# NVIDIA/cuopt

Hardware: AMD Instinct MI355X
Metric: pdlp_iterations_per_sec (higher is better)
Workload: dtype f64; 1 GPU; c3: synthetic random sparse LP S(m=1000000,n=1000000,k=10,seed=2), nnz=10000000, longest row 10, CSR fp64/int32, Stable2 preset, tolerances 0 (fixed iteration budget); rows=1000000, cols=1000000, nnz=10000000, parallelism=single GPU

## Files before the change

### cuopt_amd/csrc/kernels_layout_build.hip

```cpp
#include <hip/hip_runtime.h>

#include "pdlp_setup.hpp"
#include "setup_primitives.hpp"

namespace {

__global__ void __launch_bounds__(kT) k_panel_count(const int32_t* __restrict__ row0, const int32_t* __restrict__ off,
                                                    const int32_t* __restrict__ idx, int S, int32_t slab_w, int64_t own_from,
                                                    int32_t* __restrict__ count )
{
  __shared__ int c[16];
  if (threadIdx.x < 16) c[threadIdx.x] = 0;
  __syncthreads();
  const int w = blockIdx.x;
  const int32_t a = row0[w], b = row0[w + 1];
  for (int32_t i = a + threadIdx.x; i < b; i += kT) {
    const int32_t k0 = off[i], k1 = off[i + 1];
    if ((int64_t)(k1 - k0) > own_from) continue;
    int s_cur = -1, run = 0;
    for (int32_t k = k0; k < k1; ++k) {
      const int s2 = idx[k] / slab_w;
      if (s2 != s_cur) {
        if (run) atomicAdd(&c[s_cur], run);
        s_cur = s2, run = 0;
// ... 95 lines not shown
                        const int32_t* d_off, const int32_t* d_idx, const double* d_val, int64_t slab_bytes, bool force)
{
  PanelHost h;
  std::vector<char> is_own;
  int64_t own_nnz = 0, own_from = 0;
  const bool timing = getenv("CUOPT_AMD_TIMING") != nullptr;
  auto t_last = std::chrono::steady_clock::now();
  auto plap = [&](const char* what) {
    if (!timing) return;
    const auto now = std::chrono::steady_clock::now();
    fprintf(stderr, "[cuopt_amd setup]     panels: %-18s %6.2f ms\n", what, 1e3 * std::chrono::duration<double>(now - t_last).count());
    t_last = now;
  };
  if (!panel_plan(&h, rows, cols, h_off, slab_bytes, force, nullptr, &is_own, &own_nnz, &own_from)) return 0;
  plap("plan");
  const int W = h.W, S = h.S;
  const int64_t nnz = h_off[rows];
  h.nnz = (size_t)(nnz - own_nnz), h.rowptr_size = h.seg ? 0 : (size_t)S * ((size_t)rows + W);
  int32_t *row0 = nullptr, *tile_ptr = nullptr, *col = nullptr, *count = nullptr;
  uint16_t* rowptr = nullptr;
  int64_t* rp_base = nullptr;
  TRY(upload_i32(c, &row0, h.row0.data(), h.row0.size()));
  TRY(dev_alloc(c, &count, (size_t)W * S + 1));
  k_panel_count<<<W, kT, 0, c->stream>>>(row0, d_off, d_idx, S, h.slab_w, own_from, count);
  std::vector<int32_t> hc((size_t)W * S);
  HIP_TRY(hipMemcpyAsync(hc.data(), count, hc.size() * sizeof(int32_t), hipMemcpyDeviceToHost, c->stream));
  HIP_TRY(hipStreamSynchronize(c->stream));
  plap("count");
  h.tile_ptr.resize((size_t)W * S + 1);
  int64_t pos = 0;
  for (size_t i = 0; i < (size_t)W * S; ++i) {
    if (!h.seg && hc[i] >= 65536) return 0;
    if (hc[i] >= 65536) return 1;
    h.tile_ptr[i] = (int32_t)pos;
    pos += hc[i];
  }
  h.tile_ptr[(size_t)W * S] = (int32_t)pos;
  h.rp_base.assign((size_t)W * S, 0);
  if (!h.seg)
    for (int w = 0; w < W; ++w) {
      const int64_t a = h.row0[w], nr = h.row0[w + 1] - a, rp = (int64_t)S * (a + w);
      for (int s2 = 0; s2 < S; ++s2) h.rp_base[(size_t)w * S + s2] = rp + (int64_t)s2 * (nr + 1);
    }
  TRY(upload_i32(c, &tile_ptr, h.tile_ptr.data(), h.tile_ptr.size()));
  {
    auto pad = [](size_t b) { return (b + 255) & ~(size_t)255; };
    const size_t b_col = pad((h.nnz + 8) * sizeof(int32_t)), b_rp = pad((h.rowptr_size + 8) * sizeof(uint16_t)), b_val = pad((h.nnz + 8) * sizeof(double));
    char* block = nullptr;
    HIP_TRY(hipMalloc((void**)&block, 2 * b_col + b_rp + b_val));
    c->allocs.push_back(block);
    c->bytes += (int64_t)(2 * b_col + b_rp + b_val);
    dst->val  = (double*)block;
    col       = (int32_t*)(block + b_val);
    dst->perm = (int32_t*)(block + b_val + b_col);
    rowptr    = (uint16_t*)(block + b_val + 2 * b_col);
  }
  TRY(dev_alloc(c, &rp_base, h.rp_base.size()));
  HIP_TRY(hipMemcpyAsync(rp_base, h.rp_base.data(), h.rp_base.size() * sizeof(int64_t), hipMemcpyHostToDevice, c->stream));
  plap("alloc");
  {
    const size_t lds = (size_t)S * (kPanelMaxRows + 1) * sizeof(unsigned short);
    static std::mutex mu;
    static std::vector<int> done;
    {
      std::lock_guard<std::mutex> lock(mu);
      if (std::find(done.begin(), done.end(), c->device) == done.end()) {
        HIP_TRY(hipFuncSetAttribute((const void*)k_panel_place<false>, hipFuncAttributeMaxDynamicSharedMemorySize, 16 * (kPanelMaxRows + 1) * 2));
        HIP_TRY(hipFuncSetAttribute((const void*)k_panel_place<true>, hipFuncAttributeMaxDynamicSharedMemorySize, 16 * (kPanelMaxRows + 1) * 2));
        done.push_back(c->device);
      }
    }
    if (h.seg) k_panel_place<true><<<W, 512, lds, c->stream>>>(row0, d_off, d_idx, S, h.slab_w, own_from, tile_ptr, rp_base, rowptr, dst->perm, col);
    else k_panel_place<false><<<W, 512, lds, c->stream>>>(row0, d_off, d_idx, S, h.slab_w, own_from, tile_ptr, rp_base, rowptr, dst->perm, col);
    HIP_TRY(hipGetLastError());
    if (h.sorted) {
      k_panel_sort<<<W * S, 512, 0, c->stream>>>(S, h.slab_w, tile_ptr, dst->perm, col);
      HIP_TRY(hipGetLastError());
    }
  }
  HIP_TRY(hipStreamSynchronize(c->stream));
  plap("place");
  dst->v = PanelView{h.W, h.S, h.any_long ? 1 : 0, row0, tile_ptr, rowptr, rp_base, col, dst->val};
  dst->v.seg = h.seg ? 1 : 0, dst->v.slab_w = h.slab_w, dst->v.sorted = h.sorted ? 1 : 0;
  dst->nent  = (int64_t)h.nnz;
  if (!h.own_row.empty()) {
    int32_t *own_row = nullptr, *own_ptr = nullptr;
    TRY(upload_i32(c, &own_row, h.own_row.data(), h.own_row.size()));
    TRY(upload_i32(c, &own_ptr, h.own_ptr.data(), h.own_ptr.size()));
    HIP_TRY(hipStreamSynchronize(c->stream));
    dst->v.NP = h.W, dst->v.W = h.W + (int)h.own_row.size();
    dst->v.own_row = own_row, dst->v.own_ptr = own_ptr;
    dst->v.csr_off = d_off, dst->v.csr_idx = d_idx, dst->v.csr_val = d_val;
  }
  dst->on = true;
  return 0;
}

namespace {
constexpr int kPbBinT  = 1024;
constexpr int kPbSortN = 16384;
static_assert(kPbCap <= kPbSortN && kPbMaxRows <= 1024, "a bin's entries / rows fit the LDS sorts");

__global__ void __launch_bounds__(kT) k_max_row_len(int32_t rows, const int32_t* __restrict__ off, int* __restrict__ out)
{
  int best = 0;
  for (int64_t r = (int64_t)blockIdx.x * kT + threadIdx.x; r < rows; r += (int64_t)gridDim.x * kT) best = max(best, off[r + 1] - off[r]);
  for (int d = 1; d < 64; d <<= 1) best = max(best, __shfl_xor(best, d, 64));
  if ((threadIdx.x & 63) == 0 && best > 0) atomicMax(out, best);
}

constexpr int kPbItems = (kPbCap + kPbBinT - 1) / kPbBinT;
template <int MODE>
__global__ void __launch_bounds__(kPbBinT)
k_pb_bin(const int32_t* __restrict__ row0, const int32_t* __restrict__ off, const int32_t* __restrict__ idx, int panel_shift, int gshift, int S, int B,
         int32_t* __restrict__ bin_size, int* __restrict__ maxpad, uint16_t* __restrict__ cnt, const int32_t* __restrict__ pstart,
         const int32_t* __restrict__ bin_e0, int32_t* __restrict__ perm, uint16_t* __restrict__ lidx, int32_t* __restrict__ piece_dst,
         uint16_t* __restrict__ epos)
{
  __shared__ uint32_t w[kPbSortN];
  __shared__ int scratch[kPbBinT / 64 + 1];
  const int b = blockIdx.x, tid = threadIdx.x;
  const int r0 = row0[b], r1 = row0[b + 1];
  const int k0 = off[r0], n = off[r1] - k0;
  int n2 = 1;
  while (n2 < n) n2 <<= 1;
  for (int i = tid; i < n2; i += kPbBinT) w[i] = i < n ? ((uint32_t)(idx[k0 + i] >> panel_shift) << 14 | (uint32_t)i) : 0xFFFFFFFFu;
  __syncthreads();
  lds_bitonic_sort<kPbBinT>(w, n2);
  const int G = 1 << gshift;
  const int p0 = tid * kPbItems;
  int rs[kPbItems];
  int last = 0;
#pragma unroll
  for (int q = 0; q < kPbItems; ++q) {
    const int i = p0 + q;
    const bool start = i < n && (i == 0 || (w[i] >> 14) != (w[i - 1] >> 14));
    last  = start ? i : last;
    rs[q] = last;
  }
  const int before = block_exclusive_max<kPbBinT>(last, scratch);
#pragma unroll
  for (int q = 0; q < kPbItems; ++q) rs[q] = rs[q] > before ? rs[q] : before;
  int padv[kPbItems], sum = 0;
#pragma unroll
  for (int q = 0; q < kPbItems; ++q) {
    const int i = p0 + q;
    const bool end = i < n && (i == n - 1 || (w[i] >> 14) != (w[i + 1] >> 14));
    padv[q] = end ? (G - ((i - rs[q] + 1) & (G - 1))) & (G - 1) : 0;
    sum += padv[q];
  }
  int total = 0;
  int P = block_exclusive_scan<kPbBinT>(sum, scratch, &total);
  if (MODE <= 1) {
    if (tid == 0) {
      bin_size[b] = n + total;
      atomicMax(maxpad, n + total);
    }
    if (MODE == 0) return;
  }
#pragma unroll
  for (int q = 0; q < kPbItems; ++q) {
    const int i = p0 + q;
    if (i < n) {
      const int s_ = (int)(w[i] >> 14), e = (int)(w[i] & 0x3FFF), k = k0 + e;
      const bool end = i == n - 1 || (w[i] >> 14) != (w[i + 1] >> 14);
      if (MODE == 1) {
// ... 1049 lines not shown
```

### cuopt_amd/csrc/kernels_panel.hip

```cpp
#include <hip/hip_runtime.h>

#include "pdlp_kernel_decls.hpp"
#include "pdlp_layouts.hpp"
#include "pdlp_setup.hpp"
#include "spmv_panel.hpp"

template <bool SEG>
__global__ void __launch_bounds__(kPanelThreads)
k_panel_a_dual(PanelView P, const pdlpdev_ctl* __restrict__ ctl, const double* __restrict__ xbar,
               double* __restrict__ y0, double* __restrict__ y1, const double* __restrict__ lo,
               const double* __restrict__ hi, double* __restrict__ sumy, double* __restrict__ part, double* __restrict__ ycopy,
               const p2pdev::Push* __restrict__ push)
{
  if (!loop_active(ctl)) return;
  DualEpilogue e = DualEpilogue::make(ctl, y0, y1, lo, hi, sumy, ycopy, push);
  const bool masked = !SEG && P.zmask != nullptr && (P.zforce != 0 || ctl->zskip != 0);
  if (masked && blockIdx.x == 0 && threadIdx.x == 0)
    __hip_atomic_fetch_add(const_cast<unsigned long long*>(P.zmask) + 2 * ((size_t)(P.zcols + 127) / 128), 1ull, __ATOMIC_RELAXED, __HIP_MEMORY_SCOPE_AGENT);
  panel_block_zs<SEG>(P, xbar, e, part, masked);
  if (push) p2pdev::count_exchange(push);
}

template <bool SEG>
__global__ void __launch_bounds__(kPanelThreads)
// ... 293 lines not shown
    P.tile_ptr[i] = (int32_t)pos;
    pos += count[i];
  }
  P.tile_ptr[(size_t)W * S] = (int32_t)pos;
  P.nnz = (size_t)(nnz - own_nnz), P.rowptr_size = P.seg ? 0 : (size_t)S * ((size_t)rows + W);
  P.perm.reset(P.nnz), P.col.reset(P.nnz);
  if (P.seg) {
    cuopt_amd::parallel_tasks(W, [&](int w) {
      const int32_t a = P.row0[w], b = P.row0[w + 1];
      std::vector<int32_t> cursor(S);
      for (int s2 = 0; s2 < S; ++s2) cursor[s2] = P.tile_ptr[(size_t)w * S + s2];
      for (int32_t i = a; i < b; ++i) {
        if (is_own[i]) continue;
        for (int32_t t = off[i]; t < off[i + 1]; ++t) {
          const int s2    = idx[t] / slab_w;
          const int32_t q = cursor[s2]++;
          P.perm[q] = t, P.col[q] = (int32_t)(((uint32_t)(i - a) << kSegColBits) | (uint32_t)(idx[t] - s2 * slab_w));
        }
      }
    }, nnz);
    P.ok = true;
    return P;
  }
  P.rowptr.reset(P.rowptr_size);
  P.rp_base.resize((size_t)W * S);
  cuopt_amd::parallel_tasks(W, [&](int w) {
    const int32_t a = P.row0[w], b = P.row0[w + 1], nr = b - a;
    const int64_t rp = (int64_t)S * ((int64_t)a + w);
    std::vector<int32_t> cursor(S);
    for (int s2 = 0; s2 < S; ++s2) {
      cursor[s2]                    = P.tile_ptr[(size_t)w * S + s2];
      P.rp_base[(size_t)w * S + s2] = rp + (int64_t)s2 * (nr + 1);
    }
    for (int32_t i = a; i < b; ++i) {
      for (int s2 = 0; s2 < S; ++s2)
        P.rowptr[(size_t)(P.rp_base[(size_t)w * S + s2] + (i - a))] = (uint16_t)(cursor[s2] - P.tile_ptr[(size_t)w * S + s2]);
      if (is_own[i]) continue;
      for (int32_t t = off[i]; t < off[i + 1]; ++t) {
        const int s2 = idx[t] / slab_w;
        const int32_t q = cursor[s2]++;
        P.perm[q] = t, P.col[q] = idx[t];
      }
    }
    for (int s2 = 0; s2 < S; ++s2)
      P.rowptr[(size_t)(P.rp_base[(size_t)w * S + s2] + nr)] = (uint16_t)(cursor[s2] - P.tile_ptr[(size_t)w * S + s2]);
    if (!P.sorted) return;
    std::vector<uint32_t> key;
    std::vector<int32_t> pm;
    for (int s2 = 0; s2 < S; ++s2)
      for (int32_t c0 = P.tile_ptr[(size_t)w * S + s2], t1 = P.tile_ptr[(size_t)w * S + s2 + 1]; c0 < t1; c0 += kPanelChunk) {
        const int32_t len = std::min<int32_t>(kPanelChunk, t1 - c0);
        key.resize((size_t)len), pm.assign(&P.perm[c0], &P.perm[c0] + len);
        for (int32_t i = 0; i < len; ++i) key[i] = ((uint32_t)(P.col[c0 + i] - s2 * slab_w) << 12) | (uint32_t)i;
        std::sort(key.begin(), key.end());
        for (int32_t i = 0; i < len; ++i) {
          const uint32_t slot = key[i] & 0xFFFu;
          P.col[c0 + i] = (int32_t)((slot << kSegColBits) | (key[i] >> 12)), P.perm[c0 + i] = pm[slot];
        }
      }
  }, nnz);
  P.ok = true;
  return P;
}

int upload_panels(pdlpdev_ctx* c, pdlpdev_ctx::Panels* dst, const PanelHost& h, const int32_t* d_off, const int32_t* d_idx,
                         const double* d_val)
{
  if (!h.ok) return 0;
  int32_t *row0 = nullptr, *tile_ptr = nullptr, *col = nullptr;
  uint16_t* rowptr = nullptr;
  int64_t* rp_base = nullptr;
  TRY(upload_i32(c, &row0, h.row0.data(), h.row0.size()));
  TRY(upload_i32(c, &tile_ptr, h.tile_ptr.data(), h.tile_ptr.size()));
  TRY(upload_i32(c, &col, h.col.get(), h.nnz));
  TRY(upload_i32(c, &dst->perm, h.perm.get(), h.nnz));
  TRY(dev_alloc(c, &rowptr, h.rowptr_size));
  HIP_TRY(hipMemcpyAsync(rowptr, h.rowptr.get(), h.rowptr_size * sizeof(uint16_t), hipMemcpyHostToDevice, c->stream));
  TRY(dev_alloc(c, &rp_base, h.rp_base.size()));
  HIP_TRY(hipMemcpyAsync(rp_base, h.rp_base.data(), h.rp_base.size() * sizeof(int64_t), hipMemcpyHostToDevice, c->stream));
  TRY(dev_alloc(c, &dst->val, h.nnz));
  HIP_TRY(hipStreamSynchronize(c->stream));
  dst->v  = PanelView{h.W, h.S, h.any_long ? 1 : 0, row0, tile_ptr, rowptr, rp_base, col, dst->val};
  dst->v.seg = h.seg ? 1 : 0, dst->v.slab_w = h.slab_w, dst->v.sorted = h.sorted ? 1 : 0;
  dst->nent = (int64_t)h.nnz;
  if (!h.own_row.empty()) {
    int32_t *own_row = nullptr, *own_ptr = nullptr;
    TRY(upload_i32(c, &own_row, h.own_row.data(), h.own_row.size()));
    TRY(upload_i32(c, &own_ptr, h.own_ptr.data(), h.own_ptr.size()));
    HIP_TRY(hipStreamSynchronize(c->stream));
    dst->v.NP = h.W, dst->v.W = h.W + (int)h.own_row.size();
    dst->v.own_row = own_row, dst->v.own_ptr = own_ptr;
    dst->v.csr_off = d_off, dst->v.csr_idx = d_idx, dst->v.csr_val = d_val;
  }
  dst->on = true;
  return 0;
}

int pick_layout(pdlpdev_ctx* c, pdlpdev_ctx::MatrixSide* side, const double* vec, double* out)
{
  pdlpdev_ctx::Panels* pn = &side->pan;
  if (!pn->on) return 0;
  hipEvent_t e0, e1;
  HIP_TRY(hipEventCreate(&e0));
  HIP_TRY(hipEventCreate(&e1));
  float ms_stream = 1e30f, ms_panel = 1e30f;
  for (int round = 0; round < 2; ++round)
    for (int which = 0; which < 2; ++which) {
      for (int rep = 0; rep < 4; ++rep) {
        if (rep == 1) HIP_TRY(hipEventRecord(e0, c->stream));
        if (which == 0)
          k_spmv_plain<<<stream_grid(side->nb), kBlock, 0, c->stream>>>(side->nb, side->rb, side->hot.off, side->hot.idx, side->hot.val, vec, out, (const double*)nullptr);
        else
          (pn->v.seg ? k_panel_plain<true> : k_panel_plain<false>)<<<pn->v.W, kPanelThreads, 0, c->stream>>>(pn->v, vec, out);
      }
      HIP_TRY(hipEventRecord(e1, c->stream));
      HIP_TRY(hipEventSynchronize(e1));
      float ms = 0.f;
      HIP_TRY(hipEventElapsedTime(&ms, e0, e1));
      if (which == 0)
        ms_stream = std::min(ms_stream, ms);
      else
        ms_panel = std::min(ms_panel, ms);
    }
  (void)hipEventDestroy(e0), (void)hipEventDestroy(e1);
  if (getenv("CUOPT_AMD_TIMING"))
    fprintf(stderr, "[cuopt_amd setup]   layout %-3s: stream %.1f us, panels %.1f us -> %s\n", side->name, ms_stream * 1e3 / 3,
            ms_panel * 1e3 / 3, ms_stream <= ms_panel ? "stream" : "panels");
  if (ms_stream <= ms_panel) pn->on = false;
  return 0;
}
```

### cuopt_amd/csrc/pdlp_kernels.hpp

```cpp
#pragma once
#include <hip/hip_runtime.h>
#include <stdint.h>


#include "cuopt_amd/pdlp_device.h"

namespace pdlp {

typedef double vec4d __attribute__((ext_vector_type(4)));
typedef int vec4i __attribute__((ext_vector_type(4)));

constexpr int kBlock    = 256;
constexpr int kNnzTile  = 2048;
constexpr int kNnzBlock = kNnzTile - 4;
constexpr int kLongRow  = 128;
constexpr int kMaxRowsPerBlock = 1024;

template <int XOR_MASK>
__device__ __forceinline__ double swizzle_xor(double v)
{
  static_assert(XOR_MASK >= 1 && XOR_MASK <= 16, "ds_swizzle works inside 32 lanes");
  constexpr int pattern = (XOR_MASK << 10) | 0x1F;
  int lo = __double2loint(v), hi = __double2hiint(v);
  lo = __builtin_amdgcn_ds_swizzle(lo, pattern);
// ... 48 lines not shown
  int lo = __double2loint(v), hi = __double2hiint(v);
  lo = __builtin_amdgcn_update_dpp(0, lo, CTRL, 0xf, 0xf, false);
  hi = __builtin_amdgcn_update_dpp(0, hi, CTRL, 0xf, 0xf, false);
  return __hiloint2double(hi, lo);
}
__device__ __forceinline__ double row16_sum(double v)
{
  v = v + dpp_move<0xB1>(v);
  v = v + dpp_move<0x4E>(v);
  v = v + dpp_move<0x141>(v);
  v = v + dpp_move<0x140>(v);
  return v;
}
__device__ __forceinline__ double read_lane(double v, int lane)
{
  const int lo = __builtin_amdgcn_readlane(__double2loint(v), lane);
  const int hi = __builtin_amdgcn_readlane(__double2hiint(v), lane);
  return __hiloint2double(hi, lo);
}
__device__ __forceinline__ double wave_sum_dpp(double v)
{
  v = row16_sum(v);
  return ((read_lane(v, 0) + read_lane(v, 16)) + read_lane(v, 32)) + read_lane(v, 48);
}
template <int NQ, int WAVES>
__device__ __forceinline__ void block_sum_fast(double (&v)[NQ], double* scratch )
{
  static_assert(NQ <= 4 && WAVES <= 16, "one DPP row per quantity");
  const int lane = threadIdx.x & 63, wave = threadIdx.x >> 6;
#pragma unroll
  for (int q = 0; q < NQ; ++q) {
    const double w = wave_sum_dpp(v[q]);
    if (lane == 0) scratch[q * 16 + wave] = w;
  }
  __syncthreads();
  const int q = lane >> 4, i = lane & 15;
  double part = (q < NQ && i < WAVES) ? scratch[q * 16 + i] : 0.0;
  part        = row16_sum(part);
#pragma unroll
  for (int k = 0; k < NQ; ++k) v[k] = read_lane(part, 16 * k);
}

__device__ __forceinline__ double dense_plus(const double* __restrict__ add, int r, double v) { return add ? v + add[r] : v; }

__device__ __forceinline__ bool loop_active(const pdlpdev_ctl* ctl)
{
  return ctl->error == 0 && ctl->steps_taken < ctl->target_steps;
}
__device__ __forceinline__ bool period_reached(const pdlpdev_ctl* ctl) { return ctl->steps_taken >= ctl->target_steps; }
constexpr int kPeriodGuard = 0x100;
__device__ __forceinline__ bool period_guard_skips(const pdlpdev_ctl* ctl, int& arg)
{
  const bool guarded = (arg & kPeriodGuard) != 0;
  arg &= ~kPeriodGuard;
  return guarded && !period_reached(ctl);
}

__device__ __forceinline__ int xcd_remap(int b, int nb)
{
  const int per = (nb + 7) >> 3;
  const int v   = (b & 7) * per + (b >> 3);
  return v;
}



constexpr int kPanelThreads = 512;
constexpr int kPanelChunk   = 4096;
constexpr int kPanelMaxRows = 3584;
constexpr int kPanelWaves   = kPanelThreads / 64;

struct PanelView {
  int W, S;
  int any_long;
  const int32_t* __restrict__ row0;
  const int32_t* __restrict__ tile_ptr;
  const uint16_t* __restrict__ rowptr;
  const int64_t* __restrict__ rp_base;
  const int32_t* __restrict__ col;
  const double* __restrict__ val;
  const double* __restrict__ dense_add = nullptr;
  int seg = 0, slab_w = 0;
  int sorted = 0;
  int NP = 0;
  const int32_t* __restrict__ own_row = nullptr;
  const int32_t* __restrict__ own_ptr = nullptr;
  const int32_t* __restrict__ csr_off = nullptr;
  const int32_t* __restrict__ csr_idx = nullptr;
  const double* __restrict__ csr_val  = nullptr;
  const int32_t* __restrict__ dn_own_seg   = nullptr;
  const int32_t* __restrict__ dn_pan_ptr   = nullptr;
  const int32_t* __restrict__ dn_pan_seg   = nullptr;
  const int32_t* __restrict__ dn_seg_row   = nullptr;
  const int32_t* __restrict__ dn_seg_c0    = nullptr;
  const int32_t* __restrict__ dn_seg_len   = nullptr;
  const int32_t* __restrict__ dn_seg_ptr   = nullptr;
  const double* __restrict__ dn_val        = nullptr;
  const unsigned long long* __restrict__ zmask = nullptr;
  int zcols = 0, zforce = 0;
};
constexpr int kZsQuads        = 1152;
constexpr int kPanelOwnRow = 4096;
constexpr int kPanelDenseSegs = 32;
constexpr long long kPanelNotMine = 0x7FF8C0DEC0DEC0DELL;

constexpr int kPanelPer     = kPanelChunk / kPanelThreads;
constexpr int kPanelRowsPer = (kPanelMaxRows + kPanelThreads - 1) / kPanelThreads;
constexpr int kSegColBits = 20;
constexpr unsigned kSegColMask = (1u << kSegColBits) - 1u;
static_assert(kPanelChunk <= 1 << 12, "a sorted chunk's slot takes the 12 bits beside the column");

constexpr int kJagMaxGroup = 256;
constexpr int kJagBatchRows = 16384;
#ifndef CUOPT_AMD_JAG_U
#define CUOPT_AMD_JAG_U 8
#endif
constexpr int kJagU        = CUOPT_AMD_JAG_U;
constexpr int jag_window(int waves) { return waves == 16 ? 16384 : 8192; }
constexpr size_t jag_lds_bytes(int waves) { return sizeof(double) * (size_t)(jag_window(waves) + waves * kJagMaxGroup); }
constexpr long long kJagNotMine = 0x7FF8C0DEC0DEC0DELL;

struct JagView {
  int rows, waves, ngroups, nblk, nlong;
  const int32_t* __restrict__ row0;
  const int32_t* __restrict__ tile_e;
  const int32_t* __restrict__ tile_sr;
  const uint32_t* __restrict__ sr;
  const uint16_t* __restrict__ slot;
  const double* __restrict__ val;
  const int32_t* __restrict__ win;
  const int32_t* __restrict__ set_ptr;
  const int32_t* __restrict__ set_col;
  const int32_t* __restrict__ lr_ptr;
  const int32_t* __restrict__ lr_row;
  const int32_t* __restrict__ off;
  const int32_t* __restrict__ idx;
  const double* __restrict__ csr_val;
  const double* __restrict__ dense_add = nullptr;
};


constexpr int kPbThreads = 512;
constexpr int kPbCap     = 9088;
constexpr int kPbMaxRows = 1024;
constexpr int kPbKU      = 16;
constexpr size_t kPbLdsBytes = sizeof(double) * (size_t)(kPbCap + kPbMaxRows + 128);
typedef double pb_vec2d __attribute__((ext_vector_type(2)));
constexpr int kPbwRows     = 8192;
constexpr int kPbwStep     = 1024;
constexpr int kPbwThreads  = 1024;
constexpr int kPbwMaxLevel = 6;
constexpr int kPbwAhead    = 4;
constexpr int kPbwMaxSteps = 4096;
constexpr size_t kPbwLdsBytes = sizeof(double) * (size_t)(kPbwRows + 256) + kPbwMaxSteps;

struct PbView {
  int rows, cols, S, B, gshift, panel_shift, nwg;
  const double* __restrict__ val;
  const uint16_t* __restrict__ lidx;
  const int32_t* __restrict__ piece_dst;
  const int32_t* __restrict__ wg_e0;
  const int32_t* __restrict__ wg_panel;
  const int32_t* __restrict__ bin_row0;
  const int32_t* __restrict__ bin_e0;
  const uint32_t* __restrict__ sr;
  const int32_t* __restrict__ bin_grp;
// ... 143 lines not shown
```

### cuopt_amd/csrc/spmv_panel.hpp

```cpp
#pragma once
#include <type_traits>

#include "pdlp_kernels.hpp"

namespace pdlp {

struct PanelChunk {
  int s, c0, c1, t0;
  bool valid;
};
template <int R>
__device__ __forceinline__ void panel_load(const PanelView& P, double (&va)[kPanelPer], int (&ja)[kPanelPer], int c0, int c1)
{
#pragma unroll
  for (int u = 0; u < R; ++u) {
    int k = c0 + threadIdx.x + u * kPanelThreads;
    if (u == R - 1) k = k < c1 ? k : c1 - 1;
    va[u] = __builtin_nontemporal_load(P.val + k);
    ja[u] = __builtin_nontemporal_load(P.col + k);
  }
}
__device__ __forceinline__ void panel_decode(int word, int i, bool sorted, int slab_base, int& col, int& slot)
{
  col  = sorted ? slab_base + (int)((unsigned)word & kSegColMask) : word;
  slot = sorted ? (int)((unsigned)word >> kSegColBits) : i;
}
template <int R>
__device__ __forceinline__ void panel_products(const double* __restrict__ vec, double* prod, const double (&va)[kPanelPer],
                                               const int (&ja)[kPanelPer], int len, bool sorted, int slab_base)
{
  double x[R];
  int slot[R];
#pragma unroll
  for (int u = 0; u < R; ++u) {
    int c;
    panel_decode(ja[u], threadIdx.x + u * kPanelThreads, sorted, slab_base, c, slot[u]);
    x[u] = vec[c];
  }
#pragma unroll
  for (int u = 0; u < R; ++u) {
    const int i = threadIdx.x + u * kPanelThreads;
    if (u < R - 1 || i < len) prod[slot[u]] = va[u] * x[u];
  }
}
template <int R>
__device__ __forceinline__ void panel_products_zs(const double* __restrict__ vec, double* prod, const double (&va)[kPanelPer],
                                                  const int (&ja)[kPanelPer], int len, const unsigned* zbits, int zbase, bool sorted,
                                                  int slab_base)
{
  unsigned w[R];
  int c[R], slot[R];
#pragma unroll
  for (int u = 0; u < R; ++u) {
    panel_decode(ja[u], threadIdx.x + u * kPanelThreads, sorted, slab_base, c[u], slot[u]);
    const int wi = (c[u] >> 5) - zbase;
    w[u]         = wi < kZsQuads * 4 ? zbits[wi] : ~0u;
  }
  double x[R];
#pragma unroll
  for (int u = 0; u < R; ++u) {
    x[u] = 0.0;
    if ((w[u] >> (c[u] & 31)) & 1u) x[u] = vec[c[u]];
  }
#pragma unroll
  for (int u = 0; u < R; ++u) {
    const int i = threadIdx.x + u * kPanelThreads;
    if (u < R - 1 || i < len) prod[slot[u]] = va[u] * x[u];
  }
}
constexpr int kZsPer = (kZsQuads + kPanelThreads - 1) / kPanelThreads;
__device__ __forceinline__ int panel_zs_first_quad(const PanelView& P, int s) { return (int)(((long long)s * P.slab_w) >> 7); }
__device__ __forceinline__ void panel_zs_load(const PanelView& P, int s, uint4 (&st)[kZsPer])
{
  const long long c1 = (long long)(s + 1) * P.slab_w;
  const int last     = (int)(c1 < P.zcols ? c1 : P.zcols) - 1;
  const int q0       = panel_zs_first_quad(P, s);
  int nq             = (last >> 7) - q0 + 1;
  nq                 = nq < kZsQuads ? nq : kZsQuads;
  const uint4* __restrict__ src = reinterpret_cast<const uint4*>(P.zmask) + q0;
#pragma unroll
  for (int k = 0; k < kZsPer; ++k) {
    const int q = threadIdx.x + k * kPanelThreads;
    st[k]       = uint4{0u, 0u, 0u, 0u};
    if (q < nq) st[k] = src[q];
  }
}
__device__ __forceinline__ void panel_zs_store(uint4* zq, const uint4 (&st)[kZsPer])
{
#pragma unroll
  for (int k = 0; k < kZsPer; ++k) {
    const int q = threadIdx.x + k * kPanelThreads;
    if (q < kZsQuads) zq[q] = st[k];
  }
}
#define PANEL_DISPATCH(rounds, CALL) \
  switch (rounds) {                   \
    case 1: CALL(1); break;           \
    case 2: CALL(2); break;           \
    case 3: CALL(3); break;           \
    case 4: CALL(4); break;           \
    case 5: CALL(5); break;           \
    case 6: CALL(6); break;           \
    case 7: CALL(7); break;           \
// ... 80 lines not shown
    const int k = j - D->c0[q];
    if (k >= 0 && k < D->len[q]) add += __builtin_nontemporal_load(P.dn_val + D->ptr[q] + k) * D->y[q];
  }
  return add;
}
template <class Epi>
__device__ __forceinline__ void panel_epilogue_rows(const PanelView& P, Epi& epi, double (&acc)[Epi::NQ > 0 ? Epi::NQ : 1], const double* psum,
                                                    int first, int r0, int nr, const PanelDenseSegs* D, const double* psum2)
{
  for (int r = first; r < nr; r += kPanelThreads)
    if (__double_as_longlong(psum[r]) != kPanelNotMine) {
      double v = psum2 ? psum[r] + psum2[r] : psum[r];
      if (P.dn_pan_ptr) v = v + panel_dense_col(P, D, r0 + r);
      epi.row(r0 + r, dense_plus(P.dense_add, r0 + r, v), acc);
    }
}
template <class Epi>
__device__ __forceinline__ void panel_epilogue_partials(const PanelView& P, double* __restrict__ partials, double (&acc)[Epi::NQ > 0 ? Epi::NQ : 1],
                                                        double* red, int w)
{
  if constexpr (Epi::NQ > 0) {
    block_reduce<typename Epi::Op, Epi::NQ, kPanelWaves>(acc, red);
    if (threadIdx.x == 0) {
#pragma unroll
      for (int q = 0; q < Epi::NQ; ++q) partials[(size_t)q * P.W + w] = acc[q];
    }
  }
}
template <class Epi>
__device__ __forceinline__ void panel_epilogue(const PanelView& P, Epi& epi, double* __restrict__ partials, const double* psum, double* red,
                                               int w, int r0, int nr, const PanelDenseSegs* D,
                                               const double* psum2 = nullptr )
{
  double acc[Epi::NQ > 0 ? Epi::NQ : 1];
#pragma unroll
  for (int q = 0; q < (Epi::NQ > 0 ? Epi::NQ : 1); ++q) acc[q] = Epi::Op::identity();
  panel_epilogue_rows(P, epi, acc, psum, threadIdx.x, r0, nr, D, psum2);
  panel_epilogue_partials<Epi>(P, partials, acc, red, w);
}

constexpr int kPanelEpiDepth = 4;
template <class Epi, class = void>
struct PanelEarlyOps {
  static constexpr bool on = false;
  struct type {};
};
template <class Epi>
struct PanelEarlyOps<Epi, std::void_t<typename Epi::Ops>> {
  static constexpr bool on = true;
  using type = typename Epi::Ops;
};
template <class Epi>
__device__ __forceinline__ void panel_epilogue_request(const Epi& epi, typename Epi::Ops (&pre)[kPanelEpiDepth], int r0, int nr)
{
#pragma unroll
  for (int q = 0; q < kPanelEpiDepth; ++q) {
    int r  = threadIdx.x + q * kPanelThreads;
    r      = r < nr ? r : 0;
    pre[q] = epi.load(r0 + r);
  }
}
template <class Epi>
__device__ __forceinline__ void panel_epilogue_early(const PanelView& P, Epi& epi, double* __restrict__ partials, const double* psum, double* red,
                                                     int w, int r0, int nr, const PanelDenseSegs* D,
                                                     const typename Epi::Ops (&pre)[kPanelEpiDepth], const double* psum2 = nullptr)
{
  double acc[Epi::NQ > 0 ? Epi::NQ : 1];
#pragma unroll
  for (int q = 0; q < (Epi::NQ > 0 ? Epi::NQ : 1); ++q) acc[q] = Epi::Op::identity();
  __builtin_amdgcn_s_waitcnt(0x0F70);
#pragma unroll
  for (int q = 0; q < kPanelEpiDepth; ++q) {
    const int r = threadIdx.x + q * kPanelThreads;
    if (r < nr && __double_as_longlong(psum[r]) != kPanelNotMine) {
      double v = psum2 ? psum[r] + psum2[r] : psum[r];
      if (P.dn_pan_ptr) v = v + panel_dense_col(P, D, r0 + r);
      epi.apply(r0 + r, dense_plus(P.dense_add, r0 + r, v), pre[q], acc);
    }
  }
  panel_epilogue_rows(P, epi, acc, psum, threadIdx.x + kPanelEpiDepth * kPanelThreads, r0, nr, D, psum2);
  panel_epilogue_partials<Epi>(P, partials, acc, red, w);
}

__device__ __forceinline__ void panel_row_sums(const PanelView& P, const unsigned (&ext)[kPanelRowsPer], const double* prod, double* psum,
                                               int nr, int lo, int hi)
{
  if (!P.any_long) {
#pragma unroll
    for (int q = 0; q < kPanelRowsPer; ++q) {
      const int r = threadIdx.x + q * kPanelThreads;
      if (r < nr) {
        int a = (int)(ext[q] & 0xFFFFu), b = (int)(ext[q] >> 16);
        a = a > lo ? a : lo;
        b = b < hi ? b : hi;
        if (a < b) {
          double sum = psum[r];
          for (int k = a; k < b; ++k) sum = sum + prod[k - lo];
          psum[r] = sum;
        }
      }
    }
    return;
  }
  bool any_long = false;
#pragma unroll
  for (int q = 0; q < kPanelRowsPer; ++q) {
    const int r = threadIdx.x + q * kPanelThreads;
    if (r < nr) {
      int a = (int)(ext[q] & 0xFFFFu), b = (int)(ext[q] >> 16);
      a = a > lo ? a : lo;
      b = b < hi ? b : hi;
      if (b - a > kLongRow) {
        any_long = true;
      } else if (a < b) {
        double sum = psum[r];
        for (int k = a; k < b; ++k) sum = sum + prod[k - lo];
        psum[r] = sum;
      }
    }
  }
  if (__ballot(any_long)) {
#pragma unroll
    for (int q = 0; q < kPanelRowsPer; ++q) {
      const int r = threadIdx.x + q * kPanelThreads;
      int a = 0, b = 0;
      if (r < nr) {
        a = (int)(ext[q] & 0xFFFFu), b = (int)(ext[q] >> 16);
        a = a > lo ? a : lo;
        b = b < hi ? b : hi;
      }
      unsigned long long todo = __ballot(b - a > kLongRow);
      while (todo) {
        const int l  = __builtin_ctzll(todo);
        todo &= todo - 1;
        const int la = __builtin_amdgcn_readlane(a, l), lb = __builtin_amdgcn_readlane(b, l);
        double part  = 0.0;
        for (int k = la + (int)(threadIdx.x & 63); k < lb; k += 64) part = part + prod[k - lo];
        part = wave_reduce<SumOp>(part);
        if ((int)(threadIdx.x & 63) == l) psum[r] = psum[r] + part;
      }
    }
  }
}

template <class Epi, bool ZS = false>
__device__ __forceinline__ void panel_spmv_block(const PanelView& P, const double* __restrict__ vec,
                                                 Epi& epi, double* __restrict__ partials, const unsigned long long* zmask = nullptr)
{
  static_assert(kPanelPer == 8, "PANEL_DISPATCH enumerates 1..8 rounds");
  [[maybe_unused]] uint4* zq = nullptr;
  if constexpr (ZS) {
    __shared__ uint4 zq_s[kZsQuads];
    zq = zq_s;
  }
  const bool zon = ZS && zmask != nullptr;
  __shared__ double prod[kPanelChunk];
  __shared__ double psum[kPanelMaxRows];
  __shared__ double red[kPanelWaves * (Epi::NQ > 0 ? Epi::NQ : 1)];
  __shared__ int tile_s[17];
  __shared__ long long base_s[16];
  const int w  = blockIdx.x;
  const int NP = P.NP ? P.NP : P.W;
  if (w >= NP) {
    panel_own_row(P, vec, epi, partials, w, NP, prod);
    return;
  }
  __shared__ PanelDenseSegs dseg;
  const int r0 = P.row0[w], nr = P.row0[w + 1] - r0;
  panel_dense_prepare(P, w, vec, &dseg);
  if (threadIdx.x <= P.S) tile_s[threadIdx.x] = P.tile_ptr[w * P.S + threadIdx.x];
  if (threadIdx.x < P.S) base_s[threadIdx.x] = P.rp_base[w * P.S + threadIdx.x];
  for (int r = threadIdx.x; r < nr; r += kPanelThreads) psum[r] = 0.0;
  __syncthreads();
  if (P.own_ptr)
    for (int q = P.own_ptr[w] + (int)threadIdx.x; q < P.own_ptr[w + 1]; q += kPanelThreads) psum[P.own_row[q] - r0] = __longlong_as_double(kPanelNotMine);
  auto advance = [&](PanelChunk c) -> PanelChunk {
    if (c.valid && c.c1 < tile_s[c.s + 1]) {
      c.c0 = c.c1;
      c.c1 = c.c0 + kPanelChunk < tile_s[c.s + 1] ? c.c0 + kPanelChunk : tile_s[c.s + 1];
      return c;
    }
    int s = c.s + 1;
    while (s < P.S && tile_s[s + 1] == tile_s[s]) ++s;
    c.valid = s < P.S;
    c.s     = s;
    if (c.valid) {
      c.t0 = c.c0 = tile_s[s];
      c.c1 = c.c0 + kPanelChunk < tile_s[s + 1] ? c.c0 + kPanelChunk : tile_s[s + 1];
    }
    return c;
  };
  double va[kPanelPer];
  int ja[kPanelPer];
  unsigned ext_next[kPanelRowsPer], ext[kPanelRowsPer];
#define PANEL_ROUNDS(c) (((c).c1 - (c).c0 + kPanelThreads - 1) / kPanelThreads)
#define PANEL_CALL_LOAD(R) panel_load<R>(P, va, ja, nxt.c0, nxt.c1)
#define PANEL_CALL_PRODUCTS(R) panel_products<R>(vec, prod, va, ja, cur.c1 - cur.c0, P.sorted != 0, cur.s * P.slab_w)
#define PANEL_CALL_PRODUCTS_ZS(R) panel_products_zs<R>(vec, prod, va, ja, cur.c1 - cur.c0, reinterpret_cast<const unsigned*>(zq), panel_zs_first_quad(P, cur.s) << 2, P.sorted != 0, cur.s * P.slab_w)
#define PANEL_REQUEST(c)                                                         \
  if ((c).valid) {                                                               \
    PANEL_DISPATCH(PANEL_ROUNDS(c), PANEL_CALL_LOAD)                             \
    const uint16_t* __restrict__ rp_ = P.rowptr + base_s[(c).s];                 \
    _Pragma("unroll") for (int q = 0; q < kPanelRowsPer; ++q) {                  \
      int r_      = threadIdx.x + q * kPanelThreads;                             \
      r_          = r_ < nr ? r_ : 0;                                            \
      ext_next[q] = (unsigned)rp_[r_] | ((unsigned)rp_[r_ + 1] << 16);           \
    }                                                                            \
  }
  PanelChunk none{-1, 0, 0, 0, false};
  PanelChunk nxt = advance(none);
  PANEL_REQUEST(nxt)
  PanelChunk cur = nxt;
  if (zon && cur.valid) {
    uint4 st[kZsPer];
    panel_zs_load(P, cur.s, st);
    panel_zs_store(zq, st);
  }
  constexpr bool kEarly = PanelEarlyOps<Epi>::on;
  [[maybe_unused]] typename PanelEarlyOps<Epi>::type pre[kPanelEpiDepth];
  [[maybe_unused]] int lo_last = 0, hi_last = 0;
  while (cur.valid) {
    __syncthreads();
    if (zon) { PANEL_DISPATCH(PANEL_ROUNDS(cur), PANEL_CALL_PRODUCTS_ZS) }
    else { PANEL_DISPATCH(PANEL_ROUNDS(cur), PANEL_CALL_PRODUCTS) }
#pragma unroll
    for (int q = 0; q < kPanelRowsPer; ++q) ext[q] = ext_next[q];
    const int lo = cur.c0 - cur.t0, hi = cur.c1 - cur.t0;
    nxt = advance(cur);
    if constexpr (kEarly)
      if (!nxt.valid) {
        lo_last = lo, hi_last = hi;
        break;
      }
    PANEL_REQUEST(nxt)
    __syncthreads();
    if (zon && nxt.valid && nxt.s != cur.s) {
      uint4 st[kZsPer];
      panel_zs_load(P, nxt.s, st);
      panel_row_sums(P, ext, prod, psum, nr, lo, hi);
      panel_zs_store(zq, st);
    } else {
      panel_row_sums(P, ext, prod, psum, nr, lo, hi);
    }
    cur = nxt;
  }
#undef PANEL_REQUEST
#undef PANEL_CALL_PRODUCTS_ZS
#undef PANEL_CALL_PRODUCTS
#undef PANEL_CALL_LOAD
#undef PANEL_ROUNDS
  if constexpr (kEarly) {
    panel_epilogue_request(epi, pre, r0, nr);
    if (cur.valid) {
      __syncthreads();
      panel_row_sums(P, ext, prod, psum, nr, lo_last, hi_last);
    }
    __syncthreads();
    panel_epilogue_early(P, epi, partials, psum, red, w, r0, nr, &dseg, pre);
  } else {
    __syncthreads();
    panel_epilogue(P, epi, partials, psum, red, w, r0, nr, &dseg);
  }
}
template <int CTRL, int ROW_MASK>
__device__ __forceinline__ double seg_dpp(double v)
{
  int lo = __double2loint(v), hi = __double2hiint(v);
  lo = __builtin_amdgcn_update_dpp(0, lo, CTRL, ROW_MASK, 0xf, false);
  hi = __builtin_amdgcn_update_dpp(0, hi, CTRL, ROW_MASK, 0xf, false);
  return __hiloint2double(hi, lo);
}
__device__ __forceinline__ double seg_scan(double S, int lane, int seg0)
{
  double u;
  u = seg_dpp<0x111, 0xf>(S); if ((lane & 15) >= 1 && lane - 1 >= seg0) S = S + u;
  u = seg_dpp<0x112, 0xf>(S); if ((lane & 15) >= 2 && lane - 2 >= seg0) S = S + u;
  u = seg_dpp<0x114, 0xf>(S); if ((lane & 15) >= 4 && lane - 4 >= seg0) S = S + u;
  u = seg_dpp<0x118, 0xf>(S); if ((lane & 15) >= 8 && lane - 8 >= seg0) S = S + u;
  u = seg_dpp<0x142, 0xa>(S); if ((lane & 16) && (lane | 15) - 16 >= seg0) S = S + u;
  u = seg_dpp<0x143, 0xc>(S); if (lane >= 32 && 31 >= seg0) S = S + u;
  return S;
}
__device__ __forceinline__ void seg_emit(double* strip, int row, double v)
{
  __hip_atomic_fetch_add(strip + row, v, __ATOMIC_RELAXED, __HIP_MEMORY_SCOPE_WORKGROUP);
}
struct SegRecord {
  double lsum, rsum;
  int lkey, rkey;
};
template <int R>
__device__ __forceinline__ void seg_load(const PanelView& P, double (&va)[kPanelPer], int (&pk)[kPanelPer], int c0, int c1)
{
#pragma unroll
  for (int u = 0; u < R; ++u) {
    int k = c0 + threadIdx.x + u * kPanelThreads;
    if (u == R - 1) k = k < c1 ? k : c1 - 1;
    va[u] = __builtin_nontemporal_load(P.val + k);
    pk[u] = __builtin_nontemporal_load(P.col + k);
  }
}
template <int R>
__device__ __forceinline__ void seg_rounds(const double* __restrict__ vec, int slab_base, const double (&va)[kPanelPer], const int (&pk)[kPanelPer], int len,
                                           double* psum, SegRecord* rec , int lane)
{
  double x[R];
#pragma unroll
  for (int u = 0; u < R; ++u) x[u] = vec[slab_base + (int)((unsigned)pk[u] & kSegColMask)];
#pragma unroll
  for (int u = 0; u < R; ++u) {
    const int i   = threadIdx.x + u * kPanelThreads;
    const int key = (int)((unsigned)pk[u] >> kSegColBits);
    const double v = (u < R - 1 || i < len) ? va[u] * x[u] : 0.0;
    const int prev = __builtin_amdgcn_update_dpp(-1, key, 0x138, 0xf, 0xf, false);
    const unsigned long long starts = __ballot(key != prev);
    const unsigned long long below  = starts & ((2ull << lane) - 1ull);
    const int seg0                  = 63 - __builtin_clzll(below);
    const double S                  = seg_scan(v, lane, seg0);
    const bool ends                 = lane == 63 || ((starts >> (lane + 1)) & 1ull);
    if (ends) {
      if (seg0 == 0) {
        rec[u].lsum = S, rec[u].lkey = key;
        if (lane == 63) rec[u].rkey = -1;
      } else if (lane == 63) {
        rec[u].rsum = S, rec[u].rkey = key;
      } else {
        seg_emit(psum, key, S);
      }
    }
  }
}
__device__ __forceinline__ void panel_seg_join(const SegRecord* rec , double* psum2, int R, int lane)
{
  const int u = lane >> 3, q = lane & 7;
  const bool on = u < R;
  SegRecord g{0.0, 0.0, 0, -1};
  if (on) g = rec[q * kPanelPer + u];
  const bool single = g.rkey < 0;
// ... 128 lines not shown
```

Before: 6774 iterations/s.

## Issue panel row-extent loads before entry loads and skip unused row slots

Adds a req_order mode, on by default for non-segmented panels, that fetches row-pointer extents before the value and column loads of the next chunk. The entry loads now use clamped byte offsets and load only the rounds each chunk needs. Row-sum and extent work skips the upper row slots when the panel has few rows, and tile-pointer reads are made wave-uniform with readfirstlane. The aim is to cut load-issue latency and wasted work in the SpMV panel loop. The cost is a second instantiation of the loop body, which adds code size and register pressure.

After: 6880 iterations/s (median of 6 runs). +1.6%, better.

```diff
diff --git a/cuopt_amd/csrc/kernels_layout_build.hip b/cuopt_amd/csrc/kernels_layout_build.hip
--- a/cuopt_amd/csrc/kernels_layout_build.hip
+++ b/cuopt_amd/csrc/kernels_layout_build.hip
@@ -201,6 +201,7 @@
   plap("place");
   dst->v = PanelView{h.W, h.S, h.any_long ? 1 : 0, row0, tile_ptr, rowptr, rp_base, col, dst->val};
   dst->v.seg = h.seg ? 1 : 0, dst->v.slab_w = h.slab_w, dst->v.sorted = h.sorted ? 1 : 0;
+  dst->v.req_order = !h.seg && cuopt_amd::tune_int("panel_req_order", 1) != 0 ? 1 : 0;
   dst->nent  = (int64_t)h.nnz;
   if (!h.own_row.empty()) {
     int32_t *own_row = nullptr, *own_ptr = nullptr;
diff --git a/cuopt_amd/csrc/kernels_panel.hip b/cuopt_amd/csrc/kernels_panel.hip
--- a/cuopt_amd/csrc/kernels_panel.hip
+++ b/cuopt_amd/csrc/kernels_panel.hip
@@ -399,6 +399,7 @@
   HIP_TRY(hipStreamSynchronize(c->stream));
   dst->v  = PanelView{h.W, h.S, h.any_long ? 1 : 0, row0, tile_ptr, rowptr, rp_base, col, dst->val};
   dst->v.seg = h.seg ? 1 : 0, dst->v.slab_w = h.slab_w, dst->v.sorted = h.sorted ? 1 : 0;
+  dst->v.req_order = !h.seg && cuopt_amd::tune_int("panel_req_order", 1) != 0 ? 1 : 0;
   dst->nent = (int64_t)h.nnz;
   if (!h.own_row.empty()) {
     int32_t *own_row = nullptr, *own_ptr = nullptr;
diff --git a/cuopt_amd/csrc/pdlp_kernels.hpp b/cuopt_amd/csrc/pdlp_kernels.hpp
--- a/cuopt_amd/csrc/pdlp_kernels.hpp
+++ b/cuopt_amd/csrc/pdlp_kernels.hpp
@@ -154,6 +154,7 @@
   const double* __restrict__ dense_add = nullptr;
   int seg = 0, slab_w = 0;
   int sorted = 0;
+  int req_order = 0;
   int NP = 0;
   const int32_t* __restrict__ own_row = nullptr;
   const int32_t* __restrict__ own_ptr = nullptr;
diff --git a/cuopt_amd/csrc/spmv_panel.hpp b/cuopt_amd/csrc/spmv_panel.hpp
--- a/cuopt_amd/csrc/spmv_panel.hpp
+++ b/cuopt_amd/csrc/spmv_panel.hpp
@@ -19,6 +19,28 @@
     va[u] = __builtin_nontemporal_load(P.val + k);
     ja[u] = __builtin_nontemporal_load(P.col + k);
   }
+}
+__device__ __forceinline__ void panel_load_rounds(const PanelView& P, double (&va)[kPanelPer], int (&ja)[kPanelPer], int c0, int c1, int rounds)
+{
+  unsigned ov[kPanelPer], oc[kPanelPer];
+  const int last = c1 - c0 - 1;
+#pragma unroll
+  for (int u = 0; u < kPanelPer; ++u) {
+    int i = (int)threadIdx.x + u * kPanelThreads;
+    i     = i < last ? i : last;
+    ov[u] = (unsigned)i * 8u, oc[u] = (unsigned)i * 4u;
+    asm volatile("" : "+v"(ov[u]), "+v"(oc[u]));
+  }
+  const char* vb = reinterpret_cast<const char*>(P.val + c0);
+  const char* cb = reinterpret_cast<const char*>(P.col + c0);
+#pragma unroll
+  for (int u = 0; u < kPanelPer; ++u)
+    if (u == 0 || u < rounds) {
+      va[u] = __builtin_nontemporal_load(reinterpret_cast<const double*>(vb + ov[u]));
+      ja[u] = __builtin_nontemporal_load(reinterpret_cast<const int*>(cb + oc[u]));
+    } else {
+      va[u] = 0.0, ja[u] = 0;
+    }
 }
 __device__ __forceinline__ void panel_decode(int word, int i, bool sorted, int slab_base, int& col, int& slot)
 {
@@ -265,12 +287,15 @@
   panel_epilogue_partials<Epi>(P, partials, acc, red, w);
 }
 
+constexpr int kPanelRowsLow = 4;
+static_assert(kPanelRowsLow < kPanelRowsPer, "");
 __device__ __forceinline__ void panel_row_sums(const PanelView& P, const unsigned (&ext)[kPanelRowsPer], const double* prod, double* psum,
-                                               int nr, int lo, int hi)
+                                               int nr, int lo, int hi, int slots)
 {
   if (!P.any_long) {
 #pragma unroll
     for (int q = 0; q < kPanelRowsPer; ++q) {
+      if (q == kPanelRowsLow && slots <= kPanelRowsLow) break;
       const int r = threadIdx.x + q * kPanelThreads;
       if (r < nr) {
         int a = (int)(ext[q] & 0xFFFFu), b = (int)(ext[q] >> 16);
@@ -357,19 +382,20 @@
   __syncthreads();
   if (P.own_ptr)
     for (int q = P.own_ptr[w] + (int)threadIdx.x; q < P.own_ptr[w + 1]; q += kPanelThreads) psum[P.own_row[q] - r0] = __longlong_as_double(kPanelNotMine);
+  auto tile = [&](int i) -> int { return __builtin_amdgcn_readfirstlane(tile_s[i]); };
   auto advance = [&](PanelChunk c) -> PanelChunk {
-    if (c.valid && c.c1 < tile_s[c.s + 1]) {
+    if (c.valid && c.c1 < tile(c.s + 1)) {
       c.c0 = c.c1;
-      c.c1 = c.c0 + kPanelChunk < tile_s[c.s + 1] ? c.c0 + kPanelChunk : tile_s[c.s + 1];
+      c.c1 = c.c0 + kPanelChunk < tile(c.s + 1) ? c.c0 + kPanelChunk : tile(c.s + 1);
       return c;
     }
     int s = c.s + 1;
-    while (s < P.S && tile_s[s + 1] == tile_s[s]) ++s;
+    while (s < P.S && tile(s + 1) == tile(s)) ++s;
     c.valid = s < P.S;
     c.s     = s;
     if (c.valid) {
-      c.t0 = c.c0 = tile_s[s];
-      c.c1 = c.c0 + kPanelChunk < tile_s[s + 1] ? c.c0 + kPanelChunk : tile_s[s + 1];
+      c.t0 = c.c0 = tile(s);
+      c.c1 = c.c0 + kPanelChunk < tile(s + 1) ? c.c0 + kPanelChunk : tile(s + 1);
     }
     return c;
   };
@@ -390,43 +416,73 @@
       ext_next[q] = (unsigned)rp_[r_] | ((unsigned)rp_[r_ + 1] << 16);           \
     }                                                                            \
   }
+#define PANEL_EXTENT(q)                                                          \
+  {                                                                              \
+    int r_      = threadIdx.x + (q) * kPanelThreads;                             \
+    r_          = r_ < nr ? r_ : 0;                                              \
+    ext_next[q] = (unsigned)rp_[r_] | ((unsigned)rp_[r_ + 1] << 16);             \
+  }
+#define PANEL_REQUEST_EXT_FIRST(c)                                                                         \
+  if ((c).valid) {                                                                                         \
+    const uint16_t* __restrict__ rp_ = P.rowptr + base_s[(c).s];                                           \
+    _Pragma("unroll") for (int q = 0; q < kPanelRowsLow; ++q) PANEL_EXTENT(q)                              \
+    if (slots > kPanelRowsLow) {                                                                           \
+      _Pragma("unroll") for (int q = kPanelRowsLow; q < kPanelRowsPer; ++q) PANEL_EXTENT(q)                \
+    }                                                                                                      \
+    panel_load_rounds(P, va, ja, (c).c0, (c).c1, PANEL_ROUNDS(c));                                         \
+  }
+  const bool ext_first = P.req_order != 0;
+  const int slots      = ext_first ? (nr + kPanelThreads - 1) / kPanelThreads : kPanelRowsPer;
   PanelChunk none{-1, 0, 0, 0, false};
   PanelChunk nxt = advance(none);
-  PANEL_REQUEST(nxt)
   PanelChunk cur = nxt;
-  if (zon && cur.valid) {
-    uint4 st[kZsPer];
-    panel_zs_load(P, cur.s, st);
-    panel_zs_store(zq, st);
-  }
   constexpr bool kEarly = PanelEarlyOps<Epi>::on;
   [[maybe_unused]] typename PanelEarlyOps<Epi>::type pre[kPanelEpiDepth];
   [[maybe_unused]] int lo_last = 0, hi_last = 0;
-  while (cur.valid) {
-    __syncthreads();
-    if (zon) { PANEL_DISPATCH(PANEL_ROUNDS(cur), PANEL_CALL_PRODUCTS_ZS) }
-    else { PANEL_DISPATCH(PANEL_ROUNDS(cur), PANEL_CALL_PRODUCTS) }
-#pragma unroll
-    for (int q = 0; q < kPanelRowsPer; ++q) ext[q] = ext_next[q];
-    const int lo = cur.c0 - cur.t0, hi = cur.c1 - cur.t0;
-    nxt = advance(cur);
-    if constexpr (kEarly)
-      if (!nxt.valid) {
-        lo_last = lo, hi_last = hi;
-        break;
-      }
-    PANEL_REQUEST(nxt)
-    __syncthreads();
-    if (zon && nxt.valid && nxt.s != cur.s) {
+  auto walk = [&](auto first) __attribute__((always_inline)) {
+    constexpr bool kFirst = decltype(first)::value;
+    if constexpr (kFirst) { PANEL_REQUEST_EXT_FIRST(nxt) }
+    else { PANEL_REQUEST(nxt) }
+    if (zon && cur.valid) {
       uint4 st[kZsPer];
-      panel_zs_load(P, nxt.s, st);
-      panel_row_sums(P, ext, prod, psum, nr, lo, hi);
+      panel_zs_load(P, cur.s, st);
       panel_zs_store(zq, st);
-    } else {
-      panel_row_sums(P, ext, prod, psum, nr, lo, hi);
-    }
-    cur = nxt;
-  }
+    }
+    while (cur.valid) {
+      __syncthreads();
+      if (zon) { PANEL_DISPATCH(PANEL_ROUNDS(cur), PANEL_CALL_PRODUCTS_ZS) }
+      else { PANEL_DISPATCH(PANEL_ROUNDS(cur), PANEL_CALL_PRODUCTS) }
+#pragma unroll
+      for (int q = 0; q < kPanelRowsLow; ++q) ext[q] = ext_next[q];
+      if (!kFirst || slots > kPanelRowsLow) {
+#pragma unroll
+        for (int q = kPanelRowsLow; q < kPanelRowsPer; ++q) ext[q] = ext_next[q];
+      }
+      const int lo = cur.c0 - cur.t0, hi = cur.c1 - cur.t0;
+      nxt = advance(cur);
+      if constexpr (kEarly)
+        if (!nxt.valid) {
+          lo_last = lo, hi_last = hi;
+          break;
+        }
+      if constexpr (kFirst) { PANEL_REQUEST_EXT_FIRST(nxt) }
+      else { PANEL_REQUEST(nxt) }
+      __syncthreads();
+      if (zon && nxt.valid && nxt.s != cur.s) {
+        uint4 st[kZsPer];
+        panel_zs_load(P, nxt.s, st);
+        panel_row_sums(P, ext, prod, psum, nr, lo, hi, slots);
+        panel_zs_store(zq, st);
+      } else {
+        panel_row_sums(P, ext, prod, psum, nr, lo, hi, slots);
+      }
+      cur = nxt;
+    }
+  };
+  if (ext_first) walk(std::true_type{});
+  else walk(std::false_type{});
+#undef PANEL_REQUEST_EXT_FIRST
+#undef PANEL_EXTENT
 #undef PANEL_REQUEST
 #undef PANEL_CALL_PRODUCTS_ZS
 #undef PANEL_CALL_PRODUCTS
@@ -436,7 +492,7 @@
     panel_epilogue_request(epi, pre, r0, nr);
     if (cur.valid) {
       __syncthreads();
-      panel_row_sums(P, ext, prod, psum, nr, lo_last, hi_last);
+      panel_row_sums(P, ext, prod, psum, nr, lo_last, hi_last, slots);
     }
     __syncthreads();
     panel_epilogue_early(P, epi, partials, psum, red, w, r0, nr, &dseg, pre);
```
